# tiberiu44/TTS-Cube

Hardware: AMD Instinct MI355X
Metric: audio samples/sec (HiFi-GAN vocoder inference) (higher is better)
Workload: dtype f32 (split fp16 hi/lo x3 MFMA, fp32 accumulate)

## Files before the change

### ttscube_amd/csrc/conv1d.hip

```cpp
#include <climits>
#include <cmath>
#include <cstdlib>

#include "common.hpp"
#include "conv_f16x3_widetall.hpp"
#include "conv_kernels.hpp"

namespace ttsc {

struct PairArgs {
    const float* x;
    float* y;
    const void* w1;
    const void* w2;
    const float* b1;
    const float* b2;
    const int* len;
    float unscale1, unscale2;
    int L, d1, accumulate;
};

template <int K, int NW>
__global__ __launch_bounds__(64 * NW, (NW == 8 ? 2 : 2)) void respair32_f16x3_kernel(PairArgs a) {
    extern __shared__ __attribute__((aligned(16))) char smem_raw[];
// ... 354 lines not shown
    c->MT = pick_mt(c->CoutV);
    c->groups = groups;
    c->cin_g = cfg->in_channels / groups;
    c->cout_g = cfg->out_channels / groups;
    c->cin_tile = cfg->in_channels;
    if (groups > 1) {
        c->MT = c->cout_g >= 128 && c->cout_g % 128 == 0 ? 128 : (c->cout_g >= 64 && c->cout_g % 64 == 0 ? 64 : 32);
        if (!(c->cout_g % c->MT == 0 || c->MT % c->cout_g == 0)) {
            delete c;
            set_error("ttsc_conv1d_create: %d output channels per group do not tile into 32-row blocks", cfg->out_channels / groups);
            return TTSC_EINVAL;
        }
        c->cin_tile = (c->MT > c->cout_g ? c->MT / c->cout_g : 1) * c->cin_g;
    }
    c->NT = c->MT == 128 ? 128 : (c->MT == 64 ? 256 : 512);
    c->CinP = (int)round_up(c->cin_tile, KC);
    c->CoutP = (int)round_up(c->CoutV, c->MT);
    *out = c;
    return TTSC_OK;
}

static void free_phases(ttsc_conv1d* c) {
    for (auto& p : c->phases) {
        if (p.wp_dev) (void)hipFree(p.wp_dev);
        if (p.wph_dev) (void)hipFree(p.wph_dev);
    }
    c->phases.clear();
}

extern "C" void ttsc_conv1d_destroy(ttsc_conv1d* c) {
    if (!c) return;
    free_phases(c);
    if (c->bias_dev) (void)hipFree(c->bias_dev);
    if (c->w_plain_dev) (void)hipFree(c->w_plain_dev);
    delete c;
}

extern "C" int64_t ttsc_conv1d_out_len(const ttsc_conv1d* c, int64_t Lin) {
    if (!c) return TTSC_EINVAL;
    const auto& g = c->cfg;
    if (g.transposed) return (Lin - 1) * g.stride - 2 * g.padding + g.kernel_size;
    return Lin + 2 * g.padding - g.dilation * (g.kernel_size - 1);
}

static void pack_phase(const ttsc_conv1d* c, const float* w, const std::vector<int>& taps_k, std::vector<float>& out) {
    const auto& g = c->cfg;
    const int Cin = g.in_channels, Cout = g.out_channels, K = g.kernel_size;
    const int cipN = c->CinP / 2, cotN = c->CoutP / 32;
    out.assign((size_t)taps_k.size() * cipN * cotN * 64, 0.f);
    for (size_t j = 0; j < taps_k.size(); ++j) {
        const int k = taps_k[j];
        for (int cip = 0; cip < cipN; ++cip)
            for (int cot = 0; cot < cotN; ++cot)
                for (int lane = 0; lane < 64; ++lane) {
                    int co = cot * 32 + (lane & 31);
                    const int ci = 2 * cip + (lane >> 5);
                    int kk = k;
                    bool ok = co < c->CoutV && ci < Cin;
                    if (c->vfused) {
                        const int r = co / Cout;
                        co -= r * Cout;
                        kk = r + k * g.stride;
                        ok = ok && kk < K;
                    }
                    float v = 0.f;
                    if (c->groups > 1) {
// ... 199 lines not shown
    }
    for (const ConvPhaseGeom& pg : geom) {
        ConvPhase ph;
        static_cast<ConvPhaseGeom&>(ph) = pg;
        if (c->precision == TTSC_PREC_F16X3) {
            pack_phase_f16(c, w, ph.taps, wscale, packed_h);
            TTSC_HIP_CHECK(hipMalloc((void**)&ph.wph_dev, packed_h.size() * sizeof(_Float16)));
            TTSC_HIP_CHECK(hipMemcpy(ph.wph_dev, packed_h.data(), packed_h.size() * sizeof(_Float16), hipMemcpyHostToDevice));
        } else {
            pack_phase(c, w, ph.taps, packed);
            TTSC_HIP_CHECK(hipMalloc((void**)&ph.wp_dev, packed.size() * sizeof(float)));
            TTSC_HIP_CHECK(hipMemcpy(ph.wp_dev, packed.data(), packed.size() * sizeof(float), hipMemcpyHostToDevice));
        }
        c->phases.push_back(ph);
    }
    if (c->bias_dev) {
        (void)hipFree(c->bias_dev);
        c->bias_dev = nullptr;
    }
    if (bias) {
        TTSC_HIP_CHECK(hipMalloc((void**)&c->bias_dev, g.out_channels * sizeof(float)));
        TTSC_HIP_CHECK(hipMemcpy(c->bias_dev, bias, g.out_channels * sizeof(float), hipMemcpyHostToDevice));
    }
    if (c->w_plain_dev) {
        (void)hipFree(c->w_plain_dev);
        c->w_plain_dev = nullptr;
    }
    if (conv_wants_plain(g)) {
        TTSC_HIP_CHECK(hipMalloc((void**)&c->w_plain_dev, c->w_host.size() * sizeof(float)));
        TTSC_HIP_CHECK(hipMemcpy(c->w_plain_dev, c->w_host.data(), c->w_host.size() * sizeof(float), hipMemcpyHostToDevice));
    }
    c->w_plain_ext = nullptr;
    c->has_weight = true;
    return TTSC_OK;
}

extern "C" int ttsc_conv1d_forward(const ttsc_conv1d* c, const float* x, int32_t B, int64_t Lin, float* y,
                                   const float* resid, const ttsc_conv1d_epilogue* ep, void* stream) {
    return ttsc_conv1d_forward_ragged(c, x, B, Lin, y, resid, ep, nullptr, nullptr, stream);
}

extern "C" int32_t ttsc_conv1d_in_channels(const ttsc_conv1d* c) { return c ? c->cfg.in_channels : 0; }

extern "C" int ttsc_conv1d_set_activation_scale(ttsc_conv1d* c, float scale) {
    TTSC_REQUIRE(c, "ttsc_conv1d_set_activation_scale: null argument");
    int e = 0;
    TTSC_REQUIRE(scale > 0.f && std::isfinite(scale) && frexpf(scale, &e) == 0.5f, "ttsc_conv1d_set_activation_scale: scale must be a power of two, got %g", scale);
    c->act_scale = scale;
    return TTSC_OK;
}
extern "C" float ttsc_conv1d_get_activation_scale(const ttsc_conv1d* c) { return c ? c->act_scale : 0.f; }

extern "C" int ttsc_conv1d_set_nonfinite_flag(ttsc_conv1d* c, uint32_t* flag_dev) {
    TTSC_REQUIRE(c, "ttsc_conv1d_set_nonfinite_flag: null argument");
    c->nf_flag = flag_dev;
    return TTSC_OK;
}

namespace ttsc {
__global__ __launch_bounds__(256) void absmax_kernel(const float* __restrict__ x, long n, unsigned* __restrict__ out) {
    __shared__ float red[4];
    float m = 0.f;
    const long stride = (long)gridDim.x * blockDim.x;
    const long i0 = (long)blockIdx.x * blockDim.x + threadIdx.x;
    if ((reinterpret_cast<uintptr_t>(x) & 15) == 0) {
        const long n4 = n >> 2;
        const float4* x4 = reinterpret_cast<const float4*>(x);
        for (long i = i0; i < n4; i += stride) {
            const float4 v = x4[i];
            m = fmaxf(fmaxf(m, fmaxf(fabsf(v.x), fabsf(v.y))), fmaxf(fabsf(v.z), fabsf(v.w)));
        }
        for (long i = (n4 << 2) + i0; i < n; i += stride) m = fmaxf(m, fabsf(x[i]));
    } else {
        for (long i = i0; i < n; i += stride) m = fmaxf(m, fabsf(x[i]));
    }
#pragma unroll
    for (int off = 32; off >= 1; off >>= 1) m = fmaxf(m, __shfl_xor(m, off));
    if ((threadIdx.x & 63) == 0) red[threadIdx.x >> 6] = m;
    __syncthreads();
    if (threadIdx.x == 0) atomicMax(out, __float_as_uint(fmaxf(fmaxf(red[0], red[1]), fmaxf(red[2], red[3]))));
}
// ... 225 lines not shown
```

### ttscube_amd/csrc/conv_internal.hpp

```cpp
#pragma once
#include "common.hpp"
#include "conv_plan.hpp"

struct ConvPhase : ttsc::ConvPhaseGeom {
    float* wp_dev = nullptr;
    void* wph_dev = nullptr;
};

struct ttsc_conv1d {
    ttsc_conv1d_cfg cfg;
    int MT = 32, NT = 512, CinP = 0, CoutP = 0;
    std::vector<ConvPhase> phases;
    float* bias_dev = nullptr;
    bool has_weight = false;
    int precision = TTSC_PREC_FP32;
    bool vfused = false;
    int CoutV = 0;
    bool vrow4 = false;
    float w_unscale = 1.f;
    float act_scale = 1.f;
    std::vector<float> w_host, b_host;
    bool has_bias = false;
    bool dev_weights = false;
    const float* bias_ext = nullptr;
    float* w_plain_dev = nullptr;
    const float* w_plain_ext = nullptr;
    int groups = 1, cin_g = 0, cout_g = 0, cin_tile = 0;
    unsigned* nf_flag = nullptr;
};


#ifdef __HIPCC__
namespace ttsc {
__device__ __forceinline__ void split2_f16(float v0, float v1, unsigned& hi, unsigned& lo) {
    typedef _Float16 h2_t __attribute__((ext_vector_type(2)));
    typedef float f2_t __attribute__((ext_vector_type(2)));
    const f2_t p = {v0, v1};
    hi = __builtin_bit_cast(unsigned, __builtin_convertvector(p, h2_t));
    float l0, l1;
    asm("v_fma_mix_f32 %0, %1, -1.0, %2 op_sel:[0,0,0] op_sel_hi:[1,0,0]" : "=v"(l0) : "v"(hi), "v"(v0));
    asm("v_fma_mix_f32 %0, %1, -1.0, %2 op_sel:[1,0,0] op_sel_hi:[1,0,0]" : "=v"(l1) : "v"(hi), "v"(v1));
    const f2_t l = {l0, l1};
    lo = __builtin_bit_cast(unsigned, __builtin_convertvector(l, h2_t));
}
}
#endif
```

### ttscube_amd/csrc/resblock.hip

```cpp
#include "conv_internal.hpp"
#include "conv_kernels.hpp"

namespace ttsc {

typedef float f32x16 __attribute__((ext_vector_type(16)));
typedef float f32x4 __attribute__((ext_vector_type(4)));
typedef _Float16 half8 __attribute__((ext_vector_type(8)));
typedef _Float16 half4 __attribute__((ext_vector_type(4)));

constexpr int RB_MAXP = 3;

#ifdef TTSC_ABLATE
#define TTSC_DBG(args, bit) (((args).dbg & (bit)) != 0)
#else
#define TTSC_DBG(args, bit) false
#endif

struct ChainArgs {
    const float* x;
    float* y;
    const half8* w1[RB_MAXP];
    const half8* w2[RB_MAXP];
    const float* b1[RB_MAXP];
    const float* b2[RB_MAXP];
    float us1[RB_MAXP], us2[RB_MAXP];
    float xs[RB_MAXP], bs1[RB_MAXP];
    int d1[RB_MAXP];
    const int* len;
    int L, npairs, accumulate;
    int halo, nto;
    float* wav;
    const float* wpost;
    const float* bpost;
    float post_in_scale, post_slope, post_out_scale;
    int post_act;
    unsigned* nf_flag;
#ifdef TTSC_ABLATE
    unsigned long long* prof;
#endif
    int dbg;
};

typedef _Float16 half2v __attribute__((ext_vector_type(2)));
typedef float float2v __attribute__((ext_vector_type(2)));

template <int K, int CT>
struct ChainGeo {
    static constexpr int OMAX = (CT - 1) + 5 * ((K - 1) / 2);
    static constexpr int MARGQ = (OMAX + CT - 1) / CT + 1;
    static constexpr int MARG = (K == 3) ? 8 : (K == 7 ? 16 : 26);
};
template <int V> struct IntTag { static constexpr int value = V; };

template <int MI, int K, int CT, int NW, int WPS, int GRP = 2, int NSLOT = 2, int WM = 1, bool IL = false, bool POST = false>
__global__ __launch_bounds__(64 * NW, WPS) void rbchain_f16x3_kernel(ChainArgs a) {
    static_assert(!POST || (IL && MI == 1 && WM == 1 && CT == 4), "conv_post epilogue: 32 channels, interleaved columns");
    extern __shared__ __attribute__((aligned(16))) char smem_raw[];
    constexpr int C = 32 * MI, NCH = 2 * MI, NG = 4 * MI;
    constexpr int WN = NW / WM, MIW = MI / WM;
    static_assert(NW % WM == 0 && MI % WM == 0, "wave grid");
    constexpr int NCOL = WN * CT * 32;
    constexpr int MARG = ChainGeo<K, CT>::MARG;
    constexpr int NQ = NCOL / CT, MARGQ = ChainGeo<K, CT>::MARGQ, PQ = NQ + 2 * MARGQ;
    constexpr int PW = IL ? CT * PQ : NCOL + 2 * MARG;
    constexpr int H = (K - 1) / 2;
    typedef float fvecT __attribute__((ext_vector_type(CT == 3 ? 4 : CT)));
    static_assert(!IL || CT == 2 || CT == 4, "interleaved columns: 2 or 4 column tiles per wave");
    constexpr int NTHR = 64 * NW;
    constexpr int STEP_ITEMS = MI * 2 * 64;
    constexpr int GRP_ITEMS = GRP * STEP_ITEMS;
    constexpr int AHEAD = NSLOT - 1;
    constexpr int NS = K * NCH, NGRP = (NS + GRP - 1) / GRP;
    half8* P = reinterpret_cast<half8*>(smem_raw);
    half8* Aw = P + (size_t)NG * 2 * PW;

    const int tid = threadIdx.x, lane = tid & 63, wv = tid >> 6;
    const int half = lane >> 5, l31 = lane & 31;
    const int b = blockIdx.y;
    const int q0 = blockIdx.x * a.nto;
    const int lin = a.len ? a.len[b] : a.L;
    if (q0 >= lin) return;
#ifdef TTSC_ABLATE
    const unsigned wg_lin = blockIdx.x + gridDim.x * blockIdx.y;
#endif
    TTSC_STAMP(a, wg_lin, 0);
    TTSC_STAMP_HWID(a, wg_lin, 15);
    const int wm = wv / WN;
    const int mi0 = wm * MIW;
    const int colw = (wv % WN) * (CT * 32);
    const int pos_w = q0 - a.halo + colw + (IL ? CT * l31 : l31);
    constexpr int CSTEP = IL ? 1 : 32;
    const int qw = (wv % WN) * 32;
    const float* xb = a.x + (size_t)b * C * a.L;
    const bool vec = IL && (lin % CT == 0) && (a.L % CT == 0) && ((q0 - a.halo) % CT == 0) && (a.nto % CT == 0) &&
                     ((reinterpret_cast<uintptr_t>(a.x) | reinterpret_cast<uintptr_t>(a.y)) % (4 * CT) == 0);

    auto stage_group = [&](const half8* w, int g, int slot) __attribute__((always_inline)) {
        constexpr int NIMAX = GRP_ITEMS / 64;
        const int NI = ((NS - g * GRP < GRP ? NS - g * GRP : GRP) * STEP_ITEMS) / 64;
        if (TTSC_DBG(a, 16)) return;
#pragma unroll
        for (int i = 0; i < (NIMAX + NW - 1) / NW; ++i) {
            const int blk = wv + i * NW;
            if (blk < NI)
                __builtin_amdgcn_global_load_lds((const __attribute__((address_space(1))) void*)(w + (size_t)g * GRP_ITEMS + blk * 64 + lane),
                                                 (__attribute__((address_space(3))) void*)(Aw + slot * GRP_ITEMS + blk * 64), 16, 0, 0);
        }
    };
    auto stage_first = [&](const half8* w) __attribute__((always_inline)) {
#pragma unroll
        for (int g = 0; g < AHEAD; ++g) stage_group(w, g, g);
    };
    stage_first(a.w1[0]);

    if constexpr (IL) {
        for (int i = tid; i < NG * 2 * CT * 2 * MARGQ; i += NTHR) {
            const int row = i / (2 * MARGQ), m = i - row * (2 * MARGQ);
            half8 z;
#pragma unroll
            for (int e = 0; e < 8; ++e) z[e] = (_Float16)0.f;
            P[(size_t)row * PQ + (m < MARGQ ? m : NQ + m)] = z;
        }
    } else {
        for (int i = tid; i < NG * 2 * 2 * MARG; i += NTHR) {
            const int pl = i / (2 * MARG), m = i - pl * (2 * MARG);
            half8 z;
#pragma unroll
            for (int e = 0; e < 8; ++e) z[e] = (_Float16)0.f;
            P[(size_t)pl * PW + (m < MARG ? m : NCOL + m)] = z;
        }
    }

    f32x16 xres[MIW][CT];
    bool pok[CT];
#pragma unroll
    for (int ct = 0; ct < CT; ++ct) {
        const int pos = pos_w + ct * CSTEP;
        pok[ct] = pos >= 0 && pos < lin;
    }
    if (IL && vec) {
        int p0 = pos_w < lin - CT ? pos_w : lin - CT;
        p0 = p0 < 0 ? 0 : p0;
        const unsigned voff = (unsigned)(4 * half * a.L + p0);
#pragma unroll
        for (int mi = 0; mi < MIW; ++mi)
#pragma unroll
            for (int r = 0; r < 16; ++r) {
                const float* row = xb + (size_t)(32 * (mi0 + mi) + (r & 3) + 8 * (r >> 2)) * a.L;
                const fvecT v = TTSC_DBG(a, 8) ? fvecT(1e-3f) : *reinterpret_cast<const fvecT*>(row + voff);
#pragma unroll
                for (int ct = 0; ct < CT; ++ct) xres[mi][ct][r] = v[ct];
            }
    } else {
#pragma unroll
        for (int ct = 0; ct < CT; ++ct) {
            const int pos = pos_w + ct * CSTEP;
            int pc = pos < lin - 1 ? pos : lin - 1;
            pc = pc < 0 ? 0 : pc;
#pragma unroll
            for (int mi = 0; mi < MIW; ++mi)
#pragma unroll
                for (int r = 0; r < 16; ++r) {
                    const int ch = 32 * (mi0 + mi) + (r & 3) + 8 * (r >> 2) + 4 * half;
                    xres[mi][ct][r] = TTSC_DBG(a, 8) ? (float)(ch + pc) * 1e-3f : xb[(size_t)ch * a.L + pc];
                }
        }
    }

#ifdef TTSC_ABLATE
    if (a.prof) {
        TTSC_STAMP(a, wg_lin, 16);
        __builtin_amdgcn_s_waitcnt(0);
        TTSC_STAMP(a, wg_lin, 17);
// ... 22 lines not shown
            for (int mi = 0; mi < MIW; ++mi)
#pragma unroll
                for (int gi = 0; gi < 4; ++gi) {
                    _Float16* ph = image_ptr(mi, ct, gi);
                    const u32x2 z = {0u, 0u};
                    *reinterpret_cast<u32x2*>(ph) = z;
                    *reinterpret_cast<u32x2*>(ph + (size_t)PW * 8) = z;
                }
        }
    auto xres_to_image = [&](float s) __attribute__((always_inline)) {
#pragma unroll
        for (int mi = 0; mi < MIW; ++mi)
#pragma unroll
            for (int ct = 0; ct < CT; ++ct)
#pragma unroll
                for (int gi = 0; gi < 4; ++gi) {
                    float v[4];
#pragma unroll
                    for (int e = 0; e < 4; ++e) {
                        const float t = xres[mi][ct][4 * gi + e] * s;
                        v[e] = fmaxf(t, t * 0.1f);
                    }
                    store_split(mi, ct, gi, v[0], v[1], v[2], v[3]);
                }
    };
    const int mi0u = __builtin_amdgcn_readfirstlane(mi0);
    auto bias_tile = [&](const float* bias, float factor, int mi) __attribute__((always_inline)) -> f32x16 {
        f32x16 c;
#pragma unroll
        for (int gi = 0; gi < 4; ++gi)
#pragma unroll
            for (int e = 0; e < 4; ++e) {
                const float lo = bias[32 * (mi0u + mi) + 8 * gi + e], hi = bias[32 * (mi0u + mi) + 8 * gi + 4 + e];
                c[4 * gi + e] = (half ? hi : lo) * factor;
            }
        return c;
    };
    auto conv = [&](const half8* w, auto dtag, int d, f32x16 (&acc)[MIW][CT], const float* bias, float bfac) __attribute__((always_inline)) {
        constexpr int D = decltype(dtag)::value;
        const half8* base = IL ? P + (size_t)(half * 2) * PW + MARGQ + qw + l31 : P + (size_t)(half * 2) * PW + MARG + colw + l31 - d * ((K - 1) / 2);
        auto bfrag = [&](int s, int pl, int ct) __attribute__((always_inline)) -> const half8* {
            const int j = s / NCH, cn = s % NCH;
            if constexpr (IL) {
                const int o = ct + (j - H) * D;
                const int ph = ((o % CT) + CT) % CT, qs = (o - ph) / CT;
                return base + (size_t)(cn * 4 + pl) * PW + ph * PQ + qs;
            } else {
                return base + (size_t)(cn * 4 + pl) * PW + j * d + ct * 32;
            }
        };
        half8 Af[2][MIW][2];
        half8 Bf[2][2][CT];
        auto readA = [&](half8 (&Aq)[MIW][2], int s) __attribute__((always_inline)) {
            const half8* ap = Aw + ((s / GRP) % NSLOT) * GRP_ITEMS + (s % GRP) * STEP_ITEMS + mi0 * 128 + lane;
#pragma unroll
            for (int mi = 0; mi < MIW; ++mi) {
                Aq[mi][0] = ap[(mi * 2 + 0) * 64];
                Aq[mi][1] = ap[(mi * 2 + 1) * 64];
            }
        };
#pragma unroll
        for (int ct = 0; ct < CT; ++ct) {
            Bf[0][0][ct] = *bfrag(0, 0, ct);
            Bf[0][1][ct] = *bfrag(0, 1, ct);
        }
        constexpr int NM = 3 * MIW * CT;
#pragma unroll
// ... 64 lines not shown
        {
            const float us = a.us2[p];
#pragma unroll
            for (int mi = 0; mi < MIW; ++mi)
#pragma unroll
                for (int ct = 0; ct < CT; ++ct)
#pragma unroll
                    for (int r = 0; r < 16; ++r) xres[mi][ct][r] = __builtin_fmaf(acc[mi][ct][r], us, xres[mi][ct][r]);
        }
        if (p + 1 < a.npairs) {
            xres_to_image(a.xs[p + 1]);
            if (!TTSC_DBG(a, 2)) __syncthreads();
        }
        TTSC_STAMP(a, wg_lin, 5 + 4 * p);
    }

    if (TTSC_DBG(a, 4)) {
        float t = 0.f;
#pragma unroll
        for (int mi = 0; mi < MIW; ++mi)
#pragma unroll
            for (int ct = 0; ct < CT; ++ct) t += xres[mi][ct][0] + xres[mi][ct][9];
        if (t == 12345.678f) a.y[0] = 1.f;
        return;
    }
    int tid_f = threadIdx.x;
    asm volatile("" : "+v"(tid_f));
    const int lane_f = tid_f & 63, wv_f = tid_f >> 6;
    const int half_f = lane_f >> 5, l31_f = lane_f & 31;
    const int mi0_f = (wv_f / WN) * MIW;
    const int colw_f = (wv_f % WN) * (CT * 32);
    const int pos_w_f = q0 - a.halo + colw_f + (IL ? CT * l31_f : l31_f);
    float* yb = a.y + (size_t)b * C * a.L;
    if constexpr (POST) {
        constexpr int FOFF = 3, PWF = NCOL + 8;
        static_assert((size_t)C * PWF * 4 <= (size_t)NG * 2 * PW * 16, "conv_post staging exceeds the image area");
        float* F = reinterpret_cast<float*>(smem_raw);
        const int col0 = colw_f + CT * l31_f;
        const bool need = col0 >= a.halo - CT && col0 + CT <= a.halo + a.nto + CT;
        const bool inside = pos_w_f >= 0 && pos_w_f + CT <= lin;
        const unsigned voff = (unsigned)(4 * half_f * a.L + (inside ? pos_w_f : 0));
#pragma unroll
        for (int r = 0; r < 16; ++r) {
            const int ch0 = (r & 3) + 8 * (r >> 2);
            fvecT yv = fvecT(0.f);
            if (a.accumulate && need && inside) yv = *reinterpret_cast<const fvecT*>(yb + (size_t)ch0 * a.L + voff);
#pragma unroll
            for (int ct = 0; ct < CT; ++ct) {
                float t = (xres[0][ct][r] + yv[ct]) * a.post_in_scale;
                t = fmaxf(t, t * a.post_slope);
                F[(size_t)(ch0 + 4 * half_f) * PWF + FOFF + col0 + ct] = inside ? t : 0.f;
            }
        }
        __syncthreads();
        if (4 * tid_f < a.nto) {
            const float* win = F + FOFF + a.halo - 3 + 4 * tid_f;
            float acc4[4] = {0.f, 0.f, 0.f, 0.f};
#pragma unroll 2
            for (int ci = 0; ci < C; ++ci) {
                float w[12];
#pragma unroll
                for (int v4 = 0; v4 < 3; ++v4) {
                    const f32x4 t = *reinterpret_cast<const f32x4*>(win + (size_t)ci * PWF + 4 * v4);
                    w[4 * v4] = t[0]; w[4 * v4 + 1] = t[1]; w[4 * v4 + 2] = t[2]; w[4 * v4 + 3] = t[3];
                }
                const float* wk = a.wpost + ci * 7;
#pragma unroll
                for (int j = 0; j < 7; ++j) {
                    const float wj = wk[j];
#pragma unroll
                    for (int e = 0; e < 4; ++e) acc4[e] = fmaf(wj, w[e + j], acc4[e]);
                }
            }
            const float bv = a.bpost ? a.bpost[0] : 0.f;
            float* wb = a.wav + (size_t)b * a.L;
            const int q = q0 + 4 * tid_f;
            float res[4];
#pragma unroll
            for (int e = 0; e < 4; ++e) res[e] = apply_act((acc4[e] + bv + 0.f) * a.post_out_scale, a.post_act) + 0.f;
            if (a.nf_flag) {
                bool bad = false;
#pragma unroll
                for (int e = 0; e < 4; ++e) bad = bad || (q + e < a.L && !(fabsf(res[e]) <= 3.0e38f));
                if (bad) atomicOr(a.nf_flag, 1u);
            }
            if (q + 3 < a.L && (((uintptr_t)(wb + q)) & 15) == 0) {
                const f32x4 o = {res[0], res[1], res[2], res[3]};
                *reinterpret_cast<f32x4*>(wb + q) = o;
            } else {
#pragma unroll
                for (int e = 0; e < 4; ++e)
                    if (q + e < a.L) wb[q + e] = res[e];
            }
        }
        return;
    }
    if (IL && vec) {
        const int col0 = colw_f + CT * l31_f;
        const bool ok = col0 >= a.halo && col0 + CT <= a.halo + a.nto && pos_w_f + CT <= lin;
        const unsigned voff = (unsigned)(4 * half_f * a.L + (ok ? pos_w_f : 0));
#pragma unroll
        for (int mi = 0; mi < MIW; ++mi) {
            fvecT yv[16];
            if (a.accumulate) {
#pragma unroll
                for (int r = 0; r < 16; ++r) yv[r] = *reinterpret_cast<const fvecT*>(yb + (size_t)(32 * (mi0_f + mi) + (r & 3) + 8 * (r >> 2)) * a.L + voff);
            } else {
#pragma unroll
                for (int r = 0; r < 16; ++r) yv[r] = fvecT(0.f);
            }
#pragma unroll
            for (int r = 0; r < 16; ++r) {
                fvecT o;
#pragma unroll
                for (int ct = 0; ct < CT; ++ct) o[ct] = xres[mi][ct][r] + yv[r][ct];
                if (ok) *reinterpret_cast<fvecT*>(yb + (size_t)(32 * (mi0_f + mi) + (r & 3) + 8 * (r >> 2)) * a.L + voff) = o;
            }
        }
#ifdef TTSC_ABLATE
        if (a.prof) {
            __builtin_amdgcn_s_waitcnt(0);
            TTSC_STAMP(a, wg_lin, 14);
        }
#endif
        return;
    }
#pragma unroll
    for (int ct = 0; ct < CT; ++ct) {
        const int col = colw_f + (IL ? CT * l31_f + ct : ct * 32 + l31_f);
        const int pos = q0 - a.halo + col;
        const bool ok = col >= a.halo && col < a.halo + a.nto && pos < lin;
        const int pc = ok ? pos : 0;
#pragma unroll
        for (int mi = 0; mi < MIW; ++mi) {
            float yv[16];
            if (a.accumulate) {
#pragma unroll
                for (int r = 0; r < 16; ++r) {
                    const int ch = 32 * (mi0_f + mi) + (r & 3) + 8 * (r >> 2) + 4 * half_f;
                    yv[r] = yb[(size_t)ch * a.L + pc];
                }
            } else {
#pragma unroll
                for (int r = 0; r < 16; ++r) yv[r] = 0.f;
            }
#pragma unroll
            for (int r = 0; r < 16; ++r) {
                const int ch = 32 * (mi0_f + mi) + (r & 3) + 8 * (r >> 2) + 4 * half_f;
                if (ok) yb[(size_t)ch * a.L + pc] = xres[mi][ct][r] + yv[r];
            }
        }
    }
#ifdef TTSC_ABLATE
    if (a.prof) {
        __builtin_amdgcn_s_waitcnt(0);
        TTSC_STAMP(a, wg_lin, 14);
    }
#endif
}

#ifdef TTSC_RB_PROBE
template __global__ void rbchain_f16x3_kernel<TTSC_RB_PROBE>(ChainArgs);
}
#else
template <int MI, int K, int CT, int NW, int WPS, int GRP = 2, int NSLOT = 2, int WM = 1, bool IL = false, bool POST = false>
static int launch_chain(ChainArgs& a, int B, hipStream_t s) {
    constexpr int NCOL = (NW / WM) * CT * 32;
    constexpr int PW = IL ? CT * (NCOL / CT + 2 * ChainGeo<K, CT>::MARGQ) : NCOL + 2 * ChainGeo<K, CT>::MARG;
    constexpr size_t lds = (size_t)(4 * MI) * 2 * PW * 16 + (size_t)NSLOT * GRP * (MI * 2 * 64) * 16;
    static_assert(lds <= 160 * 1024, "activation image exceeds the LDS");
    if (POST) a.halo = (a.halo + 3 + CT - 1) / CT * CT;
    a.nto = NCOL - 2 * a.halo;
    if (IL && a.nto > 256) a.nto &= ~31;
    TTSC_REQUIRE(a.nto >= 64, "rbchain: halo %d leaves no output columns in a %d-column tile", a.halo, NCOL);
    if (int rc = ensure_full_lds((const void*)rbchain_f16x3_kernel<MI, K, CT, NW, WPS, GRP, NSLOT, WM, IL, POST>)) return rc;
    dim3 grid((unsigned)ceil_div(a.L, a.nto), (unsigned)B);
    hipLaunchKernelGGL((rbchain_f16x3_kernel<MI, K, CT, NW, WPS, GRP, NSLOT, WM, IL, POST>), grid, dim3(64 * NW), lds, s, a);
    hipError_t e = hipGetLastError();
    if (e != hipSuccess) {
        set_error("rbchain_f16x3_kernel launch failed: %s", hipGetErrorString(e));
        return TTSC_EHIP;
    }
    return TTSC_OK;
}

template <int MI, int K>
static int launch_chain_k(ChainArgs& a, int B, int shape, hipStream_t s) {
    if constexpr (MI == 4) {
        if (shape >= 10) return launch_chain<4, K, 2, 8, 2, 1, 3, 2, true>(a, B, s);
        return launch_chain<4, K, 2, 8, 2, 1, 3, 2>(a, B, s);
    }
    constexpr int G768 = K == 3 ? 6 : (K == 7 ? 7 : 11), G768W = K == 3 ? 6 : (K == 7 ? 14 : 11);
    if constexpr (MI == 1) {
        if (shape == 22) return launch_chain<1, K, 4, 8, 2, 6, 2, 1, true, true>(a, B, s);
        if (shape == 12) return launch_chain<1, K, 4, 8, 2, 6, 2, 1, true>(a, B, s);
        if (shape == 11) return launch_chain<1, K, 4, 8, 2, 2, 2, 1, true>(a, B, s);
        if (shape == 10) return launch_chain<1, K, 4, 4, 2, 2, 2, 1, true>(a, B, s);
        if (shape == 4) return launch_chain<1, K, 3, 8, 2, G768W, 2>(a, B, s);
        if (shape == 3) return launch_chain<1, K, 3, 8, 2, G768, 2>(a, B, s);
        if (shape == 2) return launch_chain<1, K, 4, 8, 2, 6, 2>(a, B, s);
        if (shape == 1) return launch_chain<1, K, 4, 8, 2>(a, B, s);
        return launch_chain<1, K, 4, 4, 2>(a, B, s);
    }
    if constexpr (MI == 2 && K == 3) {
        if (shape == 2) return launch_chain<2, K, 3, 8, 2, 6, 2, 2>(a, B, s);
    }
    if (shape == 11 || shape == 12) return launch_chain<2, K, 2, 8, 2, 2, 2, 1, true>(a, B, s);
    if (shape == 10) return launch_chain<2, K, 2, 4, 2, 2, 2, 1, true>(a, B, s);
    if (shape == 1) return launch_chain<2, K, 2, 8, 2>(a, B, s);
    return launch_chain<2, K, 2, 4, 2>(a, B, s);
}

}

using namespace ttsc;

static int chain_pair_ok(const ttsc_conv1d* c1, const ttsc_conv1d* c2, int C, int k) {
    if (!c1 || !c2) return 0;
    const auto &g1 = c1->cfg, &g2 = c2->cfg;
    if (g1.transposed || g2.transposed) return 0;
    if (g1.in_channels != C || g1.out_channels != C || g2.in_channels != C || g2.out_channels != C) return 0;
    if (g1.kernel_size != k || g2.kernel_size != k) return 0;
    if (g2.dilation != 1 || g2.padding != (k - 1) / 2 || g1.padding != g1.dilation * (k - 1) / 2) return 0;
    if (g1.dilation < 1 || g1.dilation > 5) return 0;
    if (c1->precision != TTSC_PREC_F16X3 || c2->precision != TTSC_PREC_F16X3) return 0;
    if (!c1->has_weight || !c2->has_weight || !c1->bias_dev || !c2->bias_dev || c1->dev_weights || c2->dev_weights) return 0;
    if (c1->phases.size() != 1 || c2->phases.size() != 1 || !c1->phases[0].wph_dev || !c2->phases[0].wph_dev) return 0;
    return 1;
}

extern "C" int ttsc_rbchain_supported(const ttsc_conv1d* const* convs1, const ttsc_conv1d* const* convs2, int32_t npairs) {
    if (!convs1 || !convs2 || npairs < 1 || npairs > RB_MAXP || !convs1[0]) return 0;
    const int C = convs1[0]->cfg.in_channels, k = convs1[0]->cfg.kernel_size;
    if (!(C == 32 || C == 64 || C == 128) || !(k == 3 || k == 7 || k == 11)) return 0;
    if (C == 128 && k != 3) return 0;
    int halo = 0;
    for (int p = 0; p < npairs; ++p) {
        if (!chain_pair_ok(convs1[p], convs2[p], C, k)) return 0;
        halo += (convs1[p]->cfg.dilation + 1) * (k - 1) / 2;
    }
    const int ncol = C == 32 ? 512 : 256;
    return ncol - 2 * halo >= ncol / 2 ? 1 : 0;
}

static int chain_forward(const ttsc_conv1d* const* convs1, const ttsc_conv1d* const* convs2, int32_t npairs, const float* x, int32_t B, int64_t L, float* y,
                         int32_t accumulate, const int32_t* len_dev, int32_t shape, void* stream, const ttsc_conv1d* post, const ttsc_conv1d_epilogue* post_ep,
                         float* wav);

extern "C" int ttsc_rbchain_forward(const ttsc_conv1d* const* convs1, const ttsc_conv1d* const* convs2, int32_t npairs, const float* x,
                                    int32_t B, int64_t L, float* y, int32_t accumulate, const int32_t* len_dev, int32_t shape,
                                    void* stream) {
    TTSC_REQUIRE(convs1 && convs2 && x && y, "ttsc_rbchain_forward: null argument");
    return chain_forward(convs1, convs2, npairs, x, B, L, y, accumulate, len_dev, shape, stream, nullptr, nullptr, nullptr);
}

extern "C" int ttsc_rbchain_post_supported(const ttsc_conv1d* const* convs1, const ttsc_conv1d* const* convs2, int32_t npairs, const ttsc_conv1d* post) {
    if (!post || !ttsc_rbchain_supported(convs1, convs2, npairs)) return 0;
    if (convs1[0]->cfg.in_channels != 32) return 0;
    for (int p = 0; p < npairs; ++p) {
        const int d = convs1[p]->cfg.dilation;
        if (!(d == 1 || d == 3 || d == 5)) return 0;
    }
    const auto& g = post->cfg;
    return !g.transposed && post->groups == 1 && g.in_channels == 32 && g.out_channels == 1 && g.kernel_size == 7 && g.dilation == 1 && g.padding == 3 &&
           g.stride == 1 && post->w_plain_dev && !post->dev_weights;
}

extern "C" int ttsc_rbchain_post_forward(const ttsc_conv1d* const* convs1, const ttsc_conv1d* const* convs2, int32_t npairs, const float* x, int32_t B,
                                         int64_t L, const float* ysum, const ttsc_conv1d* post, const ttsc_conv1d_epilogue* post_ep, float* wav,
                                         const int32_t* len_dev, void* stream) {
    TTSC_REQUIRE(convs1 && convs2 && x && post && wav, "ttsc_rbchain_post_forward: null argument");
    TTSC_REQUIRE(ttsc_rbchain_post_supported(convs1, convs2, npairs, post), "ttsc_rbchain_post_forward: these layers are not eligible");
    TTSC_REQUIRE(L % 4 == 0 && ((uintptr_t)x % 16 == 0) && (!ysum || (uintptr_t)ysum % 16 == 0),
                 "ttsc_rbchain_post_forward: L must be a multiple of 4 and x / ysum 16-byte aligned (got L = %lld)", (long long)L);
    TTSC_REQUIRE(!(post_ep && (post_ep->accumulate || post_ep->gate_dev)), "ttsc_rbchain_post_forward: conv_post epilogue options not available when fused");
    return chain_forward(convs1, convs2, npairs, x, B, L, const_cast<float*>(ysum), ysum ? 1 : 0, len_dev, 22, stream, post, post_ep, wav);
}

static int chain_forward(const ttsc_conv1d* const* convs1, const ttsc_conv1d* const* convs2, int32_t npairs, const float* x, int32_t B, int64_t L, float* y,
                         int32_t accumulate, const int32_t* len_dev, int32_t shape, void* stream, const ttsc_conv1d* post, const ttsc_conv1d_epilogue* post_ep,
                         float* wav) {
    TTSC_REQUIRE(ttsc_rbchain_supported(convs1, convs2, npairs), "ttsc_rbchain_forward: these layers are not eligible for the fused chain");
    TTSC_REQUIRE(x != y, "ttsc_rbchain_forward: y must not alias x");
    TTSC_REQUIRE(B > 0 && L > 0 && L < (1ll << 30), "ttsc_rbchain_forward: bad B/L");
    ChainArgs a;
    memset(&a, 0, sizeof(a));
    if (post) {
        a.wav = wav;
        a.wpost = post->w_plain_dev;
        a.bpost = post->bias_dev;
        a.post_in_scale = post_ep ? post_ep->in_scale : 1.f;
        a.post_slope = post_ep ? post_ep->in_slope : 1.f;
        a.post_out_scale = post_ep ? post_ep->out_scale : 1.f;
        a.post_act = post_ep ? post_ep->out_act : TTSC_ACT_NONE;
        a.nf_flag = post->nf_flag;
    }
    a.x = x;
    a.y = y;
    a.len = len_dev;
    a.L = (int)L;
    a.npairs = npairs;
    a.accumulate = accumulate;
#ifdef TTSC_ABLATE
    if (const char* ev = getenv("TTSC_CHAIN_DBG")) a.dbg = atoi(ev);
    if (const char* ev = getenv("TTSC_PROF_PTR")) a.prof = reinterpret_cast<unsigned long long*>(strtoull(ev, nullptr, 0));
#endif
    const int C = convs1[0]->cfg.in_channels, k = convs1[0]->cfg.kernel_size;
    for (int p = 0; p < npairs; ++p) {
        a.w1[p] = reinterpret_cast<const half8*>(convs1[p]->phases[0].wph_dev);
        a.w2[p] = reinterpret_cast<const half8*>(convs2[p]->phases[0].wph_dev);
        a.b1[p] = convs1[p]->bias_dev;
        a.b2[p] = convs2[p]->bias_dev;
        const float s1 = convs1[p]->act_scale, s2 = convs2[p]->act_scale;
        a.xs[p] = s1;
        a.us1[p] = convs1[p]->w_unscale * (s2 / s1);
        a.bs1[p] = s2;
        a.us2[p] = convs2[p]->w_unscale / s2;
        a.d1[p] = convs1[p]->cfg.dilation;
        a.halo += (a.d1[p] + 1) * (k - 1) / 2;
    }
    hipStream_t s = (hipStream_t)stream;
    bool auto_shape = false;
    if (shape < 0) {
        const int small = C == 32 ? 512 : 256;
        shape = (2 * a.halo * 6 > small) ? 1 : 0;
        if (C == 64 && (int64_t)B * ceil_div(L, 2 * small - 2 * a.halo) >= 256) shape = 1;
        auto_shape = true;
    }
    const char* il_ev = getenv("TTSC_CHAIN_IL");
    const int il_env = il_ev ? atoi(il_ev) : 1;
    bool il_ok = true;
    for (int p = 0; p < npairs; ++p) il_ok = il_ok && (a.d1[p] == 1 || a.d1[p] == 3 || a.d1[p] == 5);
    if (shape >= 10 && shape < 20 && !il_ok) shape -= 10;
    if (auto_shape && C == 32 && k == 7 && shape == 0) il_ok = false;
    if (shape >= 0 && shape <= 1 && il_env && il_ok) shape += 10;
    if (auto_shape && shape == 11 && C == 32) shape = 12;
    if (shape == 12 && !(C == 32)) shape = 11;
    if (C == 128) return launch_chain_k<4, 3>(a, B, shape, s);
    if (C == 32) {
        if (k == 3) return launch_chain_k<1, 3>(a, B, shape, s);
        if (k == 7) return launch_chain_k<1, 7>(a, B, shape, s);
        return launch_chain_k<1, 11>(a, B, shape, s);
    }
    if (k == 3) return launch_chain_k<2, 3>(a, B, shape, s);
    if (k == 7) return launch_chain_k<2, 7>(a, B, shape, s);
    return launch_chain_k<2, 11>(a, B, shape, s);
}
#endif
```

Baseline: 299.4 million.

## Add lean rbchain variant using buffer loads/stores and prescaled bias tables

Adds a LEAN template variant of the fused resblock chain kernel that is enabled by default. It replaces guarded global loads and stores with raw buffer loads and stores whose out-of-bounds offsets return zero or drop the write. It also uses scalar row offsets, buffer-to-LDS weight loads, and cached per-layer bias tables prescaled on the host so the kernel skips the bias multiply. The aim is to cut address arithmetic, VGPR use and branching in the load and epilogue paths. In exchange the code is more complex, it relies on a LEAN_OOB sentinel defined in another header, and the bias tables may force a stream sync when the scale changes.

```diff
diff --git a/ttscube_amd/csrc/conv1d.hip b/ttscube_amd/csrc/conv1d.hip
--- a/ttscube_amd/csrc/conv1d.hip
+++ b/ttscube_amd/csrc/conv1d.hip
@@ -410,6 +410,7 @@
     if (!c) return;
     free_phases(c);
     if (c->bias_dev) (void)hipFree(c->bias_dev);
+    if (c->chain_btab_dev) (void)hipFree(c->chain_btab_dev);
     if (c->w_plain_dev) (void)hipFree(c->w_plain_dev);
     delete c;
 }
@@ -675,6 +676,7 @@
     }
     c->w_plain_ext = nullptr;
     c->has_weight = true;
+    c->chain_btab_factor = 0.f;
     return TTSC_OK;
 }
 
@@ -690,6 +692,7 @@
     int e = 0;
     TTSC_REQUIRE(scale > 0.f && std::isfinite(scale) && frexpf(scale, &e) == 0.5f, "ttsc_conv1d_set_activation_scale: scale must be a power of two, got %g", scale);
     c->act_scale = scale;
+    c->chain_btab_factor = 0.f;
     return TTSC_OK;
 }
 extern "C" float ttsc_conv1d_get_activation_scale(const ttsc_conv1d* c) { return c ? c->act_scale : 0.f; }
diff --git a/ttscube_amd/csrc/conv_internal.hpp b/ttscube_amd/csrc/conv_internal.hpp
--- a/ttscube_amd/csrc/conv_internal.hpp
+++ b/ttscube_amd/csrc/conv_internal.hpp
@@ -27,6 +27,9 @@
     const float* w_plain_ext = nullptr;
     int groups = 1, cin_g = 0, cout_g = 0, cin_tile = 0;
     unsigned* nf_flag = nullptr;
+    mutable float* chain_btab_dev = nullptr;
+    mutable std::vector<float> chain_btab_host;
+    mutable float chain_btab_factor = 0.f;
 };
 
 
diff --git a/ttscube_amd/csrc/resblock.hip b/ttscube_amd/csrc/resblock.hip
--- a/ttscube_amd/csrc/resblock.hip
+++ b/ttscube_amd/csrc/resblock.hip
@@ -1,5 +1,6 @@
 #include "conv_internal.hpp"
 #include "conv_kernels.hpp"
+#include "conv_f16x3_widetall.hpp"
 
 namespace ttsc {
 
@@ -52,7 +53,7 @@
 };
 template <int V> struct IntTag { static constexpr int value = V; };
 
-template <int MI, int K, int CT, int NW, int WPS, int GRP = 2, int NSLOT = 2, int WM = 1, bool IL = false, bool POST = false>
+template <bool LEAN, int MI, int K, int CT, int NW, int WPS, int GRP = 2, int NSLOT = 2, int WM = 1, bool IL = false, bool POST = false>
 __global__ __launch_bounds__(64 * NW, WPS) void rbchain_f16x3_kernel(ChainArgs a) {
     static_assert(!POST || (IL && MI == 1 && WM == 1 && CT == 4), "conv_post epilogue: 32 channels, interleaved columns");
     extern __shared__ __attribute__((aligned(16))) char smem_raw[];
@@ -78,7 +79,8 @@
     const int half = lane >> 5, l31 = lane & 31;
     const int b = blockIdx.y;
     const int q0 = blockIdx.x * a.nto;
-    const int lin = a.len ? a.len[b] : a.L;
+    const int lin_v = a.len ? a.len[b] : a.L;
+    const int lin = LEAN ? __builtin_amdgcn_readfirstlane(lin_v) : lin_v;
     if (q0 >= lin) return;
 #ifdef TTSC_ABLATE
     const unsigned wg_lin = blockIdx.x + gridDim.x * blockIdx.y;
@@ -92,6 +94,21 @@
     constexpr int CSTEP = IL ? 1 : 32;
     const int qw = (wv % WN) * 32;
     const float* xb = a.x + (size_t)b * C * a.L;
+    const int rowb = a.L * 4;
+    const int mi0s = WM == 1 ? 0 : __builtin_amdgcn_readfirstlane(mi0);
+    const int wvs = __builtin_amdgcn_readfirstlane(wv);
+    const __amdgpu_buffer_rsrc_t xrs = __builtin_amdgcn_make_buffer_rsrc(const_cast<float*>(xb), 0, LEAN ? C * a.L * 4 : 0, 0x00020000);
+    auto row_soff = [&](int mis, int mi, int r) __attribute__((always_inline)) { return (32 * (mis + mi) + (r & 3) + 8 * (r >> 2)) * rowb; };
+    auto lean_loadv = [&](__amdgpu_buffer_rsrc_t rs, unsigned voff, int soff) __attribute__((always_inline)) -> fvecT {
+        if constexpr (CT == 2) return __builtin_bit_cast(fvecT, __builtin_amdgcn_raw_buffer_load_b64(rs, (int)voff, soff, 0));
+        else return __builtin_bit_cast(fvecT, __builtin_amdgcn_raw_buffer_load_b128(rs, (int)voff, soff, 0));
+    };
+    auto lean_storev = [&](fvecT v, __amdgpu_buffer_rsrc_t rs, unsigned voff, int soff) __attribute__((always_inline)) {
+        typedef unsigned u32x4 __attribute__((ext_vector_type(4)));
+        typedef unsigned u32x2v __attribute__((ext_vector_type(2)));
+        if constexpr (CT == 2) __builtin_amdgcn_raw_buffer_store_b64(__builtin_bit_cast(u32x2v, v), rs, (int)voff, soff, 0);
+        else __builtin_amdgcn_raw_buffer_store_b128(__builtin_bit_cast(u32x4, v), rs, (int)(voff + (unsigned)soff), 0, 0);
+    };
     const bool vec = IL && (lin % CT == 0) && (a.L % CT == 0) && ((q0 - a.halo) % CT == 0) && (a.nto % CT == 0) &&
                      ((reinterpret_cast<uintptr_t>(a.x) | reinterpret_cast<uintptr_t>(a.y)) % (4 * CT) == 0);
 
@@ -101,8 +118,13 @@
         if (TTSC_DBG(a, 16)) return;
 #pragma unroll
         for (int i = 0; i < (NIMAX + NW - 1) / NW; ++i) {
-            const int blk = wv + i * NW;
-            if (blk < NI)
+            const int blk = (LEAN ? wvs : wv) + i * NW;
+            if constexpr (LEAN) {
+                const __amdgpu_buffer_rsrc_t wrs = __builtin_amdgcn_make_buffer_rsrc(const_cast<half8*>(w), 0, NS * STEP_ITEMS * 16, 0x00020000);
+                if (blk < NI)
+                    __builtin_amdgcn_raw_ptr_buffer_load_lds(wrs, (__attribute__((address_space(3))) void*)(Aw + slot * GRP_ITEMS + blk * 64), 16, lane * 16,
+                                                             (g * GRP_ITEMS + blk * 64) * 16, 0, 0);
+            } else if (blk < NI)
                 __builtin_amdgcn_global_load_lds((const __attribute__((address_space(1))) void*)(w + (size_t)g * GRP_ITEMS + blk * 64 + lane),
                                                  (__attribute__((address_space(3))) void*)(Aw + slot * GRP_ITEMS + blk * 64), 16, 0, 0);
         }
@@ -138,7 +160,30 @@
         const int pos = pos_w + ct * CSTEP;
         pok[ct] = pos >= 0 && pos < lin;
     }
-    if (IL && vec) {
+    if constexpr (LEAN) {
+        if (IL && vec) {
+            const unsigned voff = pok[0] ? (unsigned)(4 * half * a.L + pos_w) * 4u : LEAN_OOB;
+#pragma unroll
+            for (int mi = 0; mi < MIW; ++mi)
+#pragma unroll
+                for (int r = 0; r < 16; ++r) {
+                    const fvecT v = TTSC_DBG(a, 8) ? fvecT(1e-3f) : lean_loadv(xrs, voff, row_soff(mi0s, mi, r));
+#pragma unroll
+                    for (int ct = 0; ct < CT; ++ct) xres[mi][ct][r] = v[ct];
+                }
+        } else {
+#pragma unroll
+            for (int ct = 0; ct < CT; ++ct) {
+                const int pos = pos_w + ct * CSTEP;
+                const unsigned voff = pok[ct] ? (unsigned)(4 * half * a.L + pos) * 4u : LEAN_OOB;
+#pragma unroll
+                for (int mi = 0; mi < MIW; ++mi)
+#pragma unroll
+                    for (int r = 0; r < 16; ++r)
+                        xres[mi][ct][r] = TTSC_DBG(a, 8) ? (float)(r + pos) * 1e-3f : lean_load(xrs, voff, row_soff(mi0s, mi, r));
+            }
+        }
+    } else if (IL && vec) {
         int p0 = pos_w < lin - CT ? pos_w : lin - CT;
         p0 = p0 < 0 ? 0 : p0;
         const unsigned voff = (unsigned)(4 * half * a.L + p0);
@@ -227,7 +272,7 @@
 #pragma unroll
             for (int e = 0; e < 4; ++e) {
                 const float lo = bias[32 * (mi0u + mi) + 8 * gi + e], hi = bias[32 * (mi0u + mi) + 8 * gi + 4 + e];
-                c[4 * gi + e] = (half ? hi : lo) * factor;
+                c[4 * gi + e] = LEAN ? (half ? hi : lo) : (half ? hi : lo) * factor;
             }
         return c;
     };
@@ -358,6 +403,8 @@
     const int colw_f = (wv_f % WN) * (CT * 32);
     const int pos_w_f = q0 - a.halo + colw_f + (IL ? CT * l31_f : l31_f);
     float* yb = a.y + (size_t)b * C * a.L;
+    const int mi0s_f = WM == 1 ? 0 : __builtin_amdgcn_readfirstlane(mi0_f);
+    const __amdgpu_buffer_rsrc_t yrs = __builtin_amdgcn_make_buffer_rsrc(yb, 0, LEAN && a.y ? C * a.L * 4 : 0, 0x00020000);
     if constexpr (POST) {
         constexpr int FOFF = 3, PWF = NCOL + 8;
         static_assert((size_t)C * PWF * 4 <= (size_t)NG * 2 * PW * 16, "conv_post staging exceeds the image area");
@@ -365,12 +412,14 @@
         const int col0 = colw_f + CT * l31_f;
         const bool need = col0 >= a.halo - CT && col0 + CT <= a.halo + a.nto + CT;
         const bool inside = pos_w_f >= 0 && pos_w_f + CT <= lin;
-        const unsigned voff = (unsigned)(4 * half_f * a.L + (inside ? pos_w_f : 0));
+        const unsigned voff = LEAN ? (need && inside ? (unsigned)(4 * half_f * a.L + pos_w_f) * 4u : LEAN_OOB) : (unsigned)(4 * half_f * a.L + (inside ? pos_w_f : 0));
 #pragma unroll
         for (int r = 0; r < 16; ++r) {
             const int ch0 = (r & 3) + 8 * (r >> 2);
             fvecT yv = fvecT(0.f);
-            if (a.accumulate && need && inside) yv = *reinterpret_cast<const fvecT*>(yb + (size_t)ch0 * a.L + voff);
+            if constexpr (LEAN) {
+                if (a.accumulate) yv = lean_loadv(yrs, voff, ch0 * rowb);
+            } else if (a.accumulate && need && inside) yv = *reinterpret_cast<const fvecT*>(yb + (size_t)ch0 * a.L + voff);
 #pragma unroll
             for (int ct = 0; ct < CT; ++ct) {
                 float t = (xres[0][ct][r] + yv[ct]) * a.post_in_scale;
@@ -424,13 +473,16 @@
     if (IL && vec) {
         const int col0 = colw_f + CT * l31_f;
         const bool ok = col0 >= a.halo && col0 + CT <= a.halo + a.nto && pos_w_f + CT <= lin;
-        const unsigned voff = (unsigned)(4 * half_f * a.L + (ok ? pos_w_f : 0));
+        const unsigned voff = LEAN ? (ok ? (unsigned)(4 * half_f * a.L + pos_w_f) * 4u : LEAN_OOB) : (unsigned)(4 * half_f * a.L + (ok ? pos_w_f : 0));
 #pragma unroll
         for (int mi = 0; mi < MIW; ++mi) {
             fvecT yv[16];
             if (a.accumulate) {
 #pragma unroll
-                for (int r = 0; r < 16; ++r) yv[r] = *reinterpret_cast<const fvecT*>(yb + (size_t)(32 * (mi0_f + mi) + (r & 3) + 8 * (r >> 2)) * a.L + voff);
+                for (int r = 0; r < 16; ++r) {
+                    if constexpr (LEAN) yv[r] = lean_loadv(yrs, voff, row_soff(mi0s_f, mi, r));
+                    else yv[r] = *reinterpret_cast<const fvecT*>(yb + (size_t)(32 * (mi0_f + mi) + (r & 3) + 8 * (r >> 2)) * a.L + voff);
+                }
             } else {
 #pragma unroll
                 for (int r = 0; r < 16; ++r) yv[r] = fvecT(0.f);
@@ -440,7 +492,8 @@
                 fvecT o;
 #pragma unroll
                 for (int ct = 0; ct < CT; ++ct) o[ct] = xres[mi][ct][r] + yv[r][ct];
-                if (ok) *reinterpret_cast<fvecT*>(yb + (size_t)(32 * (mi0_f + mi) + (r & 3) + 8 * (r >> 2)) * a.L + voff) = o;
+                if constexpr (LEAN) lean_storev(o, yrs, voff, row_soff(mi0s_f, mi, r));
+                else if (ok) *reinterpret_cast<fvecT*>(yb + (size_t)(32 * (mi0_f + mi) + (r & 3) + 8 * (r >> 2)) * a.L + voff) = o;
             }
         }
 #ifdef TTSC_ABLATE
@@ -457,6 +510,7 @@
         const int pos = q0 - a.halo + col;
         const bool ok = col >= a.halo && col < a.halo + a.nto && pos < lin;
         const int pc = ok ? pos : 0;
+        const unsigned voff = ok ? (unsigned)(4 * half_f * a.L + pos) * 4u : LEAN_OOB;
 #pragma unroll
         for (int mi = 0; mi < MIW; ++mi) {
             float yv[16];
@@ -464,7 +518,8 @@
 #pragma unroll
                 for (int r = 0; r < 16; ++r) {
                     const int ch = 32 * (mi0_f + mi) + (r & 3) + 8 * (r >> 2) + 4 * half_f;
-                    yv[r] = yb[(size_t)ch * a.L + pc];
+                    if constexpr (LEAN) yv[r] = lean_load(yrs, voff, row_soff(mi0s_f, mi, r));
+                    else yv[r] = yb[(size_t)ch * a.L + pc];
                 }
             } else {
 #pragma unroll
@@ -473,7 +528,8 @@
 #pragma unroll
             for (int r = 0; r < 16; ++r) {
                 const int ch = 32 * (mi0_f + mi) + (r & 3) + 8 * (r >> 2) + 4 * half_f;
-                if (ok) yb[(size_t)ch * a.L + pc] = xres[mi][ct][r] + yv[r];
+                if constexpr (LEAN) __builtin_amdgcn_raw_buffer_store_b32(__float_as_uint(xres[mi][ct][r] + yv[r]), yrs, (int)voff, row_soff(mi0s_f, mi, r), 0);
+                else if (ok) yb[(size_t)ch * a.L + pc] = xres[mi][ct][r] + yv[r];
             }
         }
     }
@@ -489,7 +545,7 @@
 template __global__ void rbchain_f16x3_kernel<TTSC_RB_PROBE>(ChainArgs);
 }
 #else
-template <int MI, int K, int CT, int NW, int WPS, int GRP = 2, int NSLOT = 2, int WM = 1, bool IL = false, bool POST = false>
+template <bool LEAN, int MI, int K, int CT, int NW, int WPS, int GRP = 2, int NSLOT = 2, int WM = 1, bool IL = false, bool POST = false>
 static int launch_chain(ChainArgs& a, int B, hipStream_t s) {
     constexpr int NCOL = (NW / WM) * CT * 32;
     constexpr int PW = IL ? CT * (NCOL / CT + 2 * ChainGeo<K, CT>::MARGQ) : NCOL + 2 * ChainGeo<K, CT>::MARG;
@@ -499,9 +555,9 @@
     a.nto = NCOL - 2 * a.halo;
     if (IL && a.nto > 256) a.nto &= ~31;
     TTSC_REQUIRE(a.nto >= 64, "rbchain: halo %d leaves no output columns in a %d-column tile", a.halo, NCOL);
-    if (int rc = ensure_full_lds((const void*)rbchain_f16x3_kernel<MI, K, CT, NW, WPS, GRP, NSLOT, WM, IL, POST>)) return rc;
+    if (int rc = ensure_full_lds((const void*)rbchain_f16x3_kernel<LEAN, MI, K, CT, NW, WPS, GRP, NSLOT, WM, IL, POST>)) return rc;
     dim3 grid((unsigned)ceil_div(a.L, a.nto), (unsigned)B);
-    hipLaunchKernelGGL((rbchain_f16x3_kernel<MI, K, CT, NW, WPS, GRP, NSLOT, WM, IL, POST>), grid, dim3(64 * NW), lds, s, a);
+    hipLaunchKernelGGL((rbchain_f16x3_kernel<LEAN, MI, K, CT, NW, WPS, GRP, NSLOT, WM, IL, POST>), grid, dim3(64 * NW), lds, s, a);
     hipError_t e = hipGetLastError();
     if (e != hipSuccess) {
         set_error("rbchain_f16x3_kernel launch failed: %s", hipGetErrorString(e));
@@ -510,31 +566,31 @@
     return TTSC_OK;
 }
 
-template <int MI, int K>
+template <int MI, int K, bool LEAN>
 static int launch_chain_k(ChainArgs& a, int B, int shape, hipStream_t s) {
     if constexpr (MI == 4) {
-        if (shape >= 10) return launch_chain<4, K, 2, 8, 2, 1, 3, 2, true>(a, B, s);
-        return launch_chain<4, K, 2, 8, 2, 1, 3, 2>(a, B, s);
+        if (shape >= 10) return launch_chain<LEAN, 4, K, 2, 8, 2, 1, 3, 2, true>(a, B, s);
+        return launch_chain<LEAN, 4, K, 2, 8, 2, 1, 3, 2>(a, B, s);
     }
     constexpr int G768 = K == 3 ? 6 : (K == 7 ? 7 : 11), G768W = K == 3 ? 6 : (K == 7 ? 14 : 11);
     if constexpr (MI == 1) {
-        if (shape == 22) return launch_chain<1, K, 4, 8, 2, 6, 2, 1, true, true>(a, B, s);
-        if (shape == 12) return launch_chain<1, K, 4, 8, 2, 6, 2, 1, true>(a, B, s);
-        if (shape == 11) return launch_chain<1, K, 4, 8, 2, 2, 2, 1, true>(a, B, s);
-        if (shape == 10) return launch_chain<1, K, 4, 4, 2, 2, 2, 1, true>(a, B, s);
-        if (shape == 4) return launch_chain<1, K, 3, 8, 2, G768W, 2>(a, B, s);
-        if (shape == 3) return launch_chain<1, K, 3, 8, 2, G768, 2>(a, B, s);
-        if (shape == 2) return launch_chain<1, K, 4, 8, 2, 6, 2>(a, B, s);
-        if (shape == 1) return launch_chain<1, K, 4, 8, 2>(a, B, s);
-        return launch_chain<1, K, 4, 4, 2>(a, B, s);
+        if (shape == 22) return launch_chain<LEAN, 1, K, 4, 8, 2, 6, 2, 1, true, true>(a, B, s);
+        if (shape == 12) return launch_chain<LEAN, 1, K, 4, 8, 2, 6, 2, 1, true>(a, B, s);
+        if (shape == 11) return launch_chain<LEAN, 1, K, 4, 8, 2, 2, 2, 1, true>(a, B, s);
+        if (shape == 10) return launch_chain<LEAN, 1, K, 4, 4, 2, 2, 2, 1, true>(a, B, s);
+        if (shape == 4) return launch_chain<LEAN, 1, K, 3, 8, 2, G768W, 2>(a, B, s);
+        if (shape == 3) return launch_chain<LEAN, 1, K, 3, 8, 2, G768, 2>(a, B, s);
+        if (shape == 2) return launch_chain<LEAN, 1, K, 4, 8, 2, 6, 2>(a, B, s);
+        if (shape == 1) return launch_chain<LEAN, 1, K, 4, 8, 2>(a, B, s);
+        return launch_chain<LEAN, 1, K, 4, 4, 2>(a, B, s);
     }
     if constexpr (MI == 2 && K == 3) {
-        if (shape == 2) return launch_chain<2, K, 3, 8, 2, 6, 2, 2>(a, B, s);
-    }
-    if (shape == 11 || shape == 12) return launch_chain<2, K, 2, 8, 2, 2, 2, 1, true>(a, B, s);
-    if (shape == 10) return launch_chain<2, K, 2, 4, 2, 2, 2, 1, true>(a, B, s);
-    if (shape == 1) return launch_chain<2, K, 2, 8, 2>(a, B, s);
-    return launch_chain<2, K, 2, 4, 2>(a, B, s);
+        if (shape == 2) return launch_chain<LEAN, 2, K, 3, 8, 2, 6, 2, 2>(a, B, s);
+    }
+    if (shape == 11 || shape == 12) return launch_chain<LEAN, 2, K, 2, 8, 2, 2, 2, 1, true>(a, B, s);
+    if (shape == 10) return launch_chain<LEAN, 2, K, 2, 4, 2, 2, 2, 1, true>(a, B, s);
+    if (shape == 1) return launch_chain<LEAN, 2, K, 2, 8, 2>(a, B, s);
+    return launch_chain<LEAN, 2, K, 2, 4, 2>(a, B, s);
 }
 
 }
@@ -601,6 +657,21 @@
                  "ttsc_rbchain_post_forward: L must be a multiple of 4 and x / ysum 16-byte aligned (got L = %lld)", (long long)L);
     TTSC_REQUIRE(!(post_ep && (post_ep->accumulate || post_ep->gate_dev)), "ttsc_rbchain_post_forward: conv_post epilogue options not available when fused");
     return chain_forward(convs1, convs2, npairs, x, B, L, const_cast<float*>(ysum), ysum ? 1 : 0, len_dev, 22, stream, post, post_ep, wav);
+}
+
+static int chain_bias_table(const ttsc_conv1d* c, float factor, hipStream_t s, const float** tab) {
+    const size_t n = (size_t)c->cfg.out_channels;
+    if (!c->chain_btab_dev || c->chain_btab_factor != factor) {
+        TTSC_REQUIRE(c->b_host.size() == n, "rbchain: layer without a host copy of its bias");
+        if (!c->chain_btab_dev) TTSC_HIP_CHECK(hipMalloc((void**)&c->chain_btab_dev, n * sizeof(float)));
+        else TTSC_HIP_CHECK(hipStreamSynchronize(s));
+        c->chain_btab_host.resize(n);
+        for (size_t i = 0; i < n; ++i) c->chain_btab_host[i] = c->b_host[i] * factor;
+        TTSC_HIP_CHECK(hipMemcpyAsync(c->chain_btab_dev, c->chain_btab_host.data(), n * sizeof(float), hipMemcpyHostToDevice, s));
+        c->chain_btab_factor = factor;
+    }
+    *tab = c->chain_btab_dev;
+    return TTSC_OK;
 }
 
 static int chain_forward(const ttsc_conv1d* const* convs1, const ttsc_conv1d* const* convs2, int32_t npairs, const float* x, int32_t B, int64_t L, float* y,
@@ -646,6 +717,13 @@
         a.halo += (a.d1[p] + 1) * (k - 1) / 2;
     }
     hipStream_t s = (hipStream_t)stream;
+    const char* lean_ev = getenv("TTSC_CHAIN_LEAN");
+    const bool lean = (!lean_ev || atoi(lean_ev) != 0) && (int64_t)C * L * 4 < (1ll << 31);
+    if (lean)
+        for (int p = 0; p < npairs; ++p) {
+            if (int rc = chain_bias_table(convs1[p], a.bs1[p] / a.us1[p], s, &a.b1[p])) return rc;
+            if (int rc = chain_bias_table(convs2[p], 1.f / a.us2[p], s, &a.b2[p])) return rc;
+        }
     bool auto_shape = false;
     if (shape < 0) {
         const int small = C == 32 ? 512 : 256;
@@ -662,14 +740,14 @@
     if (shape >= 0 && shape <= 1 && il_env && il_ok) shape += 10;
     if (auto_shape && shape == 11 && C == 32) shape = 12;
     if (shape == 12 && !(C == 32)) shape = 11;
-    if (C == 128) return launch_chain_k<4, 3>(a, B, shape, s);
+    if (C == 128) return lean ? launch_chain_k<4, 3, true>(a, B, shape, s) : launch_chain_k<4, 3, false>(a, B, shape, s);
     if (C == 32) {
-        if (k == 3) return launch_chain_k<1, 3>(a, B, shape, s);
-        if (k == 7) return launch_chain_k<1, 7>(a, B, shape, s);
-        return launch_chain_k<1, 11>(a, B, shape, s);
-    }
-    if (k == 3) return launch_chain_k<2, 3>(a, B, shape, s);
-    if (k == 7) return launch_chain_k<2, 7>(a, B, shape, s);
-    return launch_chain_k<2, 11>(a, B, shape, s);
+        if (k == 3) return lean ? launch_chain_k<1, 3, true>(a, B, shape, s) : launch_chain_k<1, 3, false>(a, B, shape, s);
+        if (k == 7) return lean ? launch_chain_k<1, 7, true>(a, B, shape, s) : launch_chain_k<1, 7, false>(a, B, shape, s);
+        return lean ? launch_chain_k<1, 11, true>(a, B, shape, s) : launch_chain_k<1, 11, false>(a, B, shape, s);
+    }
+    if (k == 3) return lean ? launch_chain_k<2, 3, true>(a, B, shape, s) : launch_chain_k<2, 3, false>(a, B, shape, s);
+    if (k == 7) return lean ? launch_chain_k<2, 7, true>(a, B, shape, s) : launch_chain_k<2, 7, false>(a, B, shape, s);
+    return lean ? launch_chain_k<2, 11, true>(a, B, shape, s) : launch_chain_k<2, 11, false>(a, B, shape, s);
 }
 #endif
```

Result: no change. 301.3 million (median of 6 runs) (+0.7%).
